# WHU-USI3DV/LaneMapping

Hardware: AMD Instinct MI355X
Metric: BEV tiles/sec end-to-end (LAS points -> polylines) (higher is better)
Workload: dtype f32

## Files before the change

include/lanemap_hip.h:

```cpp
#ifndef LANEMAP_HIP_H
#define LANEMAP_HIP_H
#include <stdint.h>
#ifdef __cplusplus
extern "C" {
#endif

enum { LM_OK = 0, LM_ERR_ARG = 1, LM_ERR_HIP = 2, LM_ERR_NO_DEVICE = 3 };
enum { LM_ACT_NONE = 0, LM_ACT_RELU = 1, LM_ACT_GELU = 2 };

int lm_abi_version(void);
const char* lm_last_error(void);
int lm_device_count(void);

int lm_conv2d_nhwc_mfma_f32(void* stream, const float* x, int ldx, const float* wp, int CoutP,
                            const float* scale, const float* shift, const float* res, int ldr, int res_rows,
                            float* y, int ldy, int B, int H, int W, int Cin, int Cout, int KH, int KW,
                            int stride, int pad_h, int pad_w, int dil, int act);
int lm_conv2d_nhwc_mfma_resup_f32(void* stream, const float* x, int ldx, const float* wp, int CoutP, const float* scale,
                                  const float* shift, const float* res_coarse, int ldr, int Hr, int Wr, float* y, int ldy,
                                  int B, int H, int W, int Cin, int Cout, int KH, int KW, int stride, int pad_h, int pad_w,
                                  int dil, int act);

int lm_winograd44_supported(int H, int W, int Cin, int dil);
int lm_winograd44_gn_chunks(int H, int W, int dil);
long lm_winograd44_tiles(int B, int H, int W, int dil);
long lm_winograd44_twin_workspace_bytes(int B, int H, int W, int Cin, int CoutP, int dil);
int lm_conv3x3_winograd44_f32(void* stream, const float* x, int ldx, const float* wu_frag, int CoutP, const float* scale,
                              const float* shift, const float* res, int ldr, float* y, int ldy, int B, int H, int W,
                              int Cin, int Cout, int dil, int act, double* gn_partial);
int lm_conv3x3_winograd44_twin_f32(void* stream, const float* x, int ldx, const float* wu, int CoutP, const float* scale,
                                   const float* shift, const float* res, int ldr, float* y, int ldy, int B, int H, int W,
                                   int Cin, int Cout, int dil, int act, void* workspace, long workspace_bytes);
int lm_wino44_split_fragments(void* stream, const float* frag, float* out, long n_quads);
int lm_conv3x3_winograd44_split_f32(void* stream, const float* x, int ldx, const float* wu_split, int CoutP, const float* scale,
                                    const float* shift, const float* res, int ldr, float* y, int ldy, int B, int H, int W,
                                    int Cin, int Cout, int dil, int act, double* gn_partial, float post);
int lm_conv3x3_winograd44_split_twin_f32(void* stream, const float* x, int ldx, const float* wu, int CoutP, const float* scale,
                                         const float* shift, const float* res, int ldr, float* y, int ldy, int B, int H, int W,
// ... 151 lines not shown
```

lanemapping_amd/_lib.py:

```python
import ctypes as C
import os

_HERE = os.path.dirname(os.path.abspath(__file__))
LIB_PATH = os.environ.get('LANEMAP_HIP_LIB') or os.path.join(_HERE, 'liblanemap_hip.so')

c_f32p = C.POINTER(C.c_float)
vp, i32, i64, f32 = C.c_void_p, C.c_int, C.c_long, C.c_float


class LmRasterParams(C.Structure):
    _fields_ = [('quat', C.c_float * 4), ('trans', C.c_float * 3), ('bev_img_offset', C.c_float * 2),
                ('img_reso', C.c_float * 2), ('local_min_ele', C.c_float), ('ele_reso', C.c_float),
                ('inten_lo', C.c_float), ('inten_hi', C.c_float)]


class LmLasHeader(C.Structure):
    _fields_ = [('version_major', C.c_int), ('version_minor', C.c_int), ('point_format', C.c_int), ('record_len', C.c_int),
                ('n_points', C.c_long), ('offset_to_points', C.c_long), ('scale', C.c_double * 3), ('offset', C.c_double * 3),
                ('min_xyz', C.c_double * 3), ('max_xyz', C.c_double * 3)]


SIGNATURES = {
    'lm_abi_version': (i32, []),
    'lm_last_error': (C.c_char_p, []),
    'lm_device_count': (i32, []),
    'lm_conv2d_nhwc_mfma_f32': (i32, [vp, vp, i32, vp, i32, vp, vp, vp, i32, i32, vp, i32,
                                      i32, i32, i32, i32, i32, i32, i32, i32, i32, i32, i32, i32]),
    'lm_conv2d_nhwc_mfma_resup_f32': (i32, [vp, vp, i32, vp, i32, vp, vp, vp, i32, i32, i32, vp, i32,
                                            i32, i32, i32, i32, i32, i32, i32, i32, i32, i32, i32, i32]),
    'lm_winograd44_supported': (i32, [i32, i32, i32, i32]),
    'lm_winograd44_gn_chunks': (i32, [i32, i32, i32]),
    'lm_winograd44_tiles': (i64, [i32, i32, i32, i32]),
    'lm_winograd44_twin_workspace_bytes': (i64, [i32, i32, i32, i32, i32, i32]),
    'lm_conv3x3_winograd44_f32': (i32, [vp, vp, i32, vp, i32, vp, vp, vp, i32, vp, i32, i32, i32, i32, i32, i32, i32, i32, vp]),
    'lm_conv3x3_winograd44_twin_f32': (i32, [vp, vp, i32, vp, i32, vp, vp, vp, i32, vp, i32, i32, i32, i32, i32, i32, i32, i32, vp, i64]),
    'lm_wino44_split_fragments': (i32, [vp, vp, vp, i64]),
    'lm_conv3x3_winograd44_split_f32': (i32, [vp, vp, i32, vp, i32, vp, vp, vp, i32, vp, i32, i32, i32, i32, i32, i32, i32, i32, vp, f32]),
    'lm_conv3x3_winograd44_split_twin_f32': (i32, [vp, vp, i32, vp, i32, vp, vp, vp, i32, vp, i32, i32, i32, i32, i32, i32, i32, i32, vp, i64, f32]),
    'lm_conv2d_nhwc_mfma_f32_gnstats': (i32, [vp, vp, i32, vp, i32, vp, vp, i32, vp] + [i32] * 11),
    'lm_gn_finalize': (i32, [vp, vp, vp, i32, i32, i32, i32, f32]),
    'lm_gn_finalize_split': (i32, [vp, vp, vp, i32, i32, i32, i32, f32, i32]),
    'lm_stem_conv7x7_bn_relu': (i32, [vp, vp, vp, vp, vp, vp, i32, i32, i32]),
    'lm_stem_conv7x7_bn_relu_u8': (i32, [vp, vp, vp, vp, vp, vp, i32, i32, i32]),
    'lm_maxpool3x3s2_nhwc': (i32, [vp, vp, vp, i32, i32, i32, i32]),
    'lm_conv2d_nhwc_small': (i32, [vp, vp, i32, vp, vp, vp, vp, i32, i32, i32, i32, i32, i32, i32, i32, i32, i32, i32, i32, i32]),
    'lm_gn_stats': (i32, [vp, vp, vp, vp, i32, i32, i32, f32]),
# ... 95 lines not shown
```

lanemapping_amd/csrc/conv_wino44.hip:

```cpp
#include "common.h"

#include <cstdlib>

typedef float f32x16 __attribute__((ext_vector_type(16)));
typedef float f32x4 __attribute__((ext_vector_type(4)));
typedef float f32x2 __attribute__((ext_vector_type(2)));
typedef _Float16 f16x4 __attribute__((ext_vector_type(4)));
typedef unsigned u32x2 __attribute__((ext_vector_type(2)));

namespace {

__device__ __forceinline__ u32x2 w44_split2(f32x2 t) {
#pragma clang fp contract(off)
    typedef __fp16 f16x2r __attribute__((ext_vector_type(2)));
    const f16x2r h = __builtin_amdgcn_cvt_pkrtz(t[0], t[1]);
    const float h0 = (float)h[0], h1 = (float)h[1];
    const f16x2r l = __builtin_amdgcn_cvt_pkrtz(t[0] - h0, t[1] - h1);
    return u32x2{__builtin_bit_cast(unsigned, h), __builtin_bit_cast(unsigned, l)};
}

constexpr int QBM = 32, QBN = 64, QSEG = 4;
constexpr int QNCELL = 144;
constexpr int QLPW = 14;
constexpr int QGRP = 256 + 8;
constexpr int QRAWF = QLPW * 4 * QGRP;
constexpr int QVF = 36 * 256;
constexpr int QBD = 5, QRING = 6;
static_assert(6 * (QNCELL / 16) * QGRP <= QRAWF && QNCELL % 16 == 0, "patch loads cover the unit");

__device__ __attribute__((aligned(16))) float g_w44_zeros[1024 + 32];

struct W44Geom {
    int B, H, W, dil, Ty, Tx;
    int Timg, Tpad;
    long T;
    LmFastDiv dTx, dTy, ddil, dTpad;
};

W44Geom geom44(int B, int H, int W, int dil) {
    W44Geom g;
    g.B = B; g.H = H; g.W = W; g.dil = dil;
    g.Ty = ((H + dil - 1) / dil + 3) / 4;
    g.Tx = ((W + dil - 1) / dil + 3) / 4;
    g.Timg = dil * dil * g.Ty * g.Tx;
    g.Tpad = (g.Timg + QBM - 1) / QBM * QBM;
    g.T = (long)B * g.Tpad;
    g.dTx = lm_fastdiv_make((unsigned)g.Tx); g.dTy = lm_fastdiv_make((unsigned)g.Ty);
    g.ddil = lm_fastdiv_make((unsigned)dil); g.dTpad = lm_fastdiv_make((unsigned)g.Tpad);
    return g;
}

__device__ __forceinline__ void tile44_decode(const W44Geom& g, int t, int& pa, int& pb, int& ty, int& tx) {
    tx = t % g.Tx;
    t /= g.Tx;
    ty = t % g.Ty;
    const int ph = t / g.Ty;
    pa = ph / g.dil;
    pb = ph - pa * g.dil;
}

// ... 188 lines not shown
    const f32x2 p = pk_fnma(d[2], k.c4, d[4]), q = pk_fnma(d[1], k.c4, d[3]);
    const f32x2 r = pk_sub(d[4], d[2]), s = pk_sub(d[3], d[1]);
    t[0] = pk_fma(d[0], k.c4, a);
    t[5] = pk_fma(d[1], k.c4, b);
    t[1] = pk_add(p, q);
    t[2] = pk_sub(p, q);
    t[3] = pk_fma(s, k.c2, r);
    t[4] = pk_fnma(s, k.c2, r);
}

struct W44Xf {
    f32x2 e[6][5];
    f32x2 w[3][6];
    f32x2 tA[6], tB[6], tC[6];
};
template <int C>
__device__ __forceinline__ void w44_preread(W44Xf& d, const float* rawrow, const int (&roff)[6]) {
    constexpr int ROWF = (QNCELL / 16) * QGRP;
    const float* s = rawrow + roff[C];
#pragma unroll
    for (int r = 0; r < 5; ++r) d.e[C][r] = *reinterpret_cast<const f32x2*>(s + r * ROWF);
}
template <bool LOWER, int C>
__device__ __forceinline__ void w44_pass1x2(W44Xf& d, const W44K& k) {
    const f32x2 (&e)[5] = d.e[C];
    const f32x2 (&f)[5] = d.e[C + 1];
    if constexpr (!LOWER) {
        const f32x2 a0 = pk_fnma(e[2], k.c5, e[4]), a1 = pk_fnma(f[2], k.c5, f[4]);
        const f32x2 p0 = pk_fnma(e[2], k.c4, e[4]), p1 = pk_fnma(f[2], k.c4, f[4]);
        const f32x2 q0 = pk_fnma(e[1], k.c4, e[3]), q1 = pk_fnma(f[1], k.c4, f[3]);
        d.w[0][C] = pk_fma(e[0], k.c4, a0);
        d.w[0][C + 1] = pk_fma(f[0], k.c4, a1);
        d.w[1][C] = pk_add(p0, q0);
        d.w[1][C + 1] = pk_add(p1, q1);
        d.w[2][C] = pk_sub(p0, q0);
        d.w[2][C + 1] = pk_sub(p1, q1);
    } else {
        const f32x2 a0 = pk_fnma(e[2], k.c5, e[4]), a1 = pk_fnma(f[2], k.c5, f[4]);
        const f32x2 r0 = pk_sub(e[3], e[1]), r1 = pk_sub(f[3], f[1]);
        const f32x2 s0 = pk_sub(e[2], e[0]), s1 = pk_sub(f[2], f[0]);
        d.w[2][C] = pk_fma(e[0], k.c4, a0);
        d.w[2][C + 1] = pk_fma(f[0], k.c4, a1);
        d.w[0][C] = pk_fma(s0, k.c2, r0);
        d.w[0][C + 1] = pk_fma(s1, k.c2, r1);
        d.w[1][C] = pk_fnma(s0, k.c2, r0);
        d.w[1][C + 1] = pk_fnma(s1, k.c2, r1);
    }
}
template <bool SPLIT>
__device__ __forceinline__ void w44_vstore(float* v, int j, const f32x2 t) {
    if constexpr (SPLIT) {
        const u32x2 w = w44_split2(t);
        reinterpret_cast<unsigned*>(v)[j * 256] = w[0];
        reinterpret_cast<unsigned*>(v)[j * 256 + 128] = w[1];
    } else {
        *reinterpret_cast<f32x2*>(v + j * 256) = t;
    }
}
template <int K, bool SPLIT>
__device__ __forceinline__ void w44_xf_lds(W44Xf& d, const float* rawrow, const int (&roff)[6], float* vA, float* vB, float* vC) {
    auto st = [](float* v, int j, const f32x2 t) { w44_vstore<SPLIT>(v, j, t); };
    if constexpr (K == 0) {
        st(vB, 2, d.tB[2]); st(vB, 5, d.tB[5]);
        w44_preread<0>(d, rawrow, roff); w44_preread<1>(d, rawrow, roff);
    } else if constexpr (K == 1) {
        st(vC, 0, d.tC[0]); st(vC, 1, d.tC[1]);
        w44_preread<2>(d, rawrow, roff); w44_preread<3>(d, rawrow, roff);
    } else if constexpr (K == 2) {
        st(vC, 2, d.tC[2]); st(vC, 3, d.tC[3]);
        w44_preread<4>(d, rawrow, roff); w44_preread<5>(d, rawrow, roff);
    } else if constexpr (K == 3) {
        st(vC, 4, d.tC[4]); st(vC, 5, d.tC[5]);
    } else if constexpr (K == 5) {
        st(vA, 0, d.tA[0]); st(vA, 1, d.tA[1]); st(vA, 2, d.tA[2]);
    } else if constexpr (K == 6) {
        st(vA, 3, d.tA[3]); st(vA, 4, d.tA[4]); st(vA, 5, d.tA[5]);
    } else if constexpr (K == 7) {
        st(vB, 0, d.tB[0]); st(vB, 1, d.tB[1]); st(vB, 3, d.tB[3]); st(vB, 4, d.tB[4]);
    }
}
template <int K>
__device__ __forceinline__ void w44_xf_valu(W44Xf& d, bool lower, const W44K& k) {
    if constexpr (K >= 1 && K <= 3) {
        if (lower) w44_pass1x2<true, 2 * K - 2>(d, k);
        else w44_pass1x2<false, 2 * K - 2>(d, k);
    } else if constexpr (K == 4) {
        pk_bt(d.w[0], d.tA, k);
    } else if constexpr (K == 5) {
        pk_bt(d.w[1], d.tB, k);
    } else if constexpr (K == 6) {
        pk_bt(d.w[2], d.tC, k);
    }
}
template <bool SPLIT>
__device__ __forceinline__ void w44_xf_all(W44Xf& d, const float* rawrow, const int (&roff)[6], float* vA, float* vB, float* vC, bool lower,
                                           const W44K& k) {
    w44_preread<0>(d, rawrow, roff); w44_preread<1>(d, rawrow, roff); w44_preread<2>(d, rawrow, roff);
    w44_preread<3>(d, rawrow, roff); w44_preread<4>(d, rawrow, roff); w44_preread<5>(d, rawrow, roff);
    w44_xf_valu<1>(d, lower, k); w44_xf_valu<2>(d, lower, k); w44_xf_valu<3>(d, lower, k);
    w44_xf_valu<4>(d, lower, k); w44_xf_valu<5>(d, lower, k); w44_xf_valu<6>(d, lower, k);
#pragma unroll
    for (int j = 0; j < 6; ++j) {
        w44_vstore<SPLIT>(vA, j, d.tA[j]);
        w44_vstore<SPLIT>(vB, j, d.tB[j]);
        w44_vstore<SPLIT>(vC, j, d.tC[j]);
    }
}

__device__ __forceinline__ void q_bload2(f32x4 (&b)[2], unsigned voff, const float* sbase) {
    asm volatile("global_load_dwordx4 %0, %2, %3\n\t"
                 "global_load_dwordx4 %1, %2, %3 offset:1024"
                 : "=&v"(b[0]), "=&v"(b[1]) : "v"(voff), "s"(sbase) : "memory");
}
template <int N>
__device__ __forceinline__ void q_bwait(f32x4 (&b)[2]) {
    asm volatile("s_waitcnt vmcnt(%2)" : "+v"(b[0]), "+v"(b[1]) : "n"(N) : "memory");
}

__device__ __forceinline__ void mfma_vgpr(f32x16& acc, float a, float b) {
    asm volatile("v_mfma_f32_32x32x2_f32 %0, %1, %2, %0" : "+v"(acc) : "v"(a), "v"(b));
// ... 38 lines not shown
    constexpr int K = S % 9;
    q_bload2(bq[(S + QBD) % QRING], bvoff, bpre);
#pragma unroll
    for (int i = 0; i < q_ndma(S); ++i) {
        constexpr int L0 = q_dma0(S);
        __builtin_amdgcn_global_load_lds((gptr_t*)(gsrc[L0 + i] + goff), (lptr_t*)(rawld + ((L0 + i) * 4 + wave) * QGRP), 16, 0, 0);
    }
    f32x4 (&b)[2] = bq[S % QRING];
    q_bwait<q_nwait(S)>(b);
    constexpr bool VACC = K == 8;
    const f32x2 a_hi = {a_cur[0], a_cur[1]}, a_lo = {a_cur[2], a_cur[3]};
    if constexpr (SPLIT) q_mfma16<VACC>(acc0, a_hi, f32x2{b[0][0], b[0][1]});
    else q_mfma<VACC>(acc0, a_cur[0], b[0][0]);
    if constexpr (!SPLIT) __builtin_amdgcn_sched_barrier(0);
    if constexpr (K != 4 && K != 8) a_nxt = q_aread<SPLIT>(anext);
    w44_xf_lds<K, SPLIT>(xf, prerow, roff, vA, vB, vC);
    if constexpr (!SPLIT) __builtin_amdgcn_sched_barrier(0);
    w44_xf_valu<K>(xf, lower, kk);
    if constexpr (!SPLIT) __builtin_amdgcn_sched_barrier(0);
    if constexpr (SPLIT) {
        q_mfma16<VACC>(acc1, a_hi, f32x2{b[1][0], b[1][1]});
        q_mfma16<VACC>(acc0, a_hi, f32x2{b[0][2], b[0][3]});
        q_mfma16<VACC>(acc1, a_hi, f32x2{b[1][2], b[1][3]});
        q_mfma16<VACC>(acc0, a_lo, f32x2{b[0][0], b[0][1]});
        q_mfma16<VACC>(acc1, a_lo, f32x2{b[1][0], b[1][1]});
        if constexpr (!VACC) {
#pragma unroll
            for (int i = 0; i < 6; ++i) {
                __builtin_amdgcn_sched_group_barrier(0x008, 1, 0);
                __builtin_amdgcn_sched_group_barrier(0x002, 6, 0);
                __builtin_amdgcn_sched_group_barrier(0x300, 3, 0);
// ... 182 lines not shown
            for (int r = 0; r < 16; ++r) acc[k][b][r] = 0.f;
    f32x4 bq[QRING][2];
    W44Xf xf;
    const int lowoff = lower ? (QNCELL / 16) * QGRP : 0;
#define LM_QXI(K) (6 * ((K) / 3) + (K) % 3)
#pragma unroll
    for (int k = 0; k < QBD; ++k) q_bload2(bq[k], bvoff, bbase + (long)LM_QXI(k) * xstride);
    {
        const long goff1 = nun > 1 ? 16 : 0;
#pragma unroll
        for (int s_ = 0; s_ < QLPW; ++s_)
            __builtin_amdgcn_global_load_lds((gptr_t*)(gsrc[s_] + goff1), (lptr_t*)(raw0 + QRAWF + (s_ * 4 + wave) * QGRP), 16, 0, 0);
    }
    q_bwait<QLPW>(bq[0]);
    __builtin_amdgcn_s_barrier();
    w44_xf_all<SPLIT>(xf, raw0 + lowoff, roff, vA, vB, vC, lower, kk);
    asm volatile("s_waitcnt lgkmcnt(0)" ::: "memory");
    __builtin_amdgcn_s_barrier();

#define LM_QBPRE(S5) ((S5) < 18 ? bu + (long)((S5) / 9) * ustride + (long)LM_QXI((S5) % 9) * xstride : bu_next + (long)LM_QXI((S5) - 18) * xstride)
#define LM_QSTEP(S, AC, AN) \
    w44_step<S, SPLIT>(acc[(S) % 9][0], acc[(S) % 9][1], bq, bvoff, LM_QBPRE((S) + QBD), Vq + LM_QXI(((S) % 9) + 1 < 9 ? ((S) % 9) + 1 : 0) * 256, \
                AC, AN, gsrc, goff, rawc_w, wave, xf, (S) < 9 ? rawc + 8 + lowoff : rawn + lowoff, roff, vA, vB, vC, lower, kk)
#define LM_QMID(AN)                                          \
    asm volatile("s_waitcnt lgkmcnt(0)" ::: "memory");       \
    __builtin_amdgcn_s_barrier();                            \
    AN = q_aread<SPLIT>(Vq + LM_QXI(5) * 256);
    for (int u = 0; u < nun; ++u) {
        const float* const rawc = raw0 + (u & 1) * QRAWF;
        float* const rawc_w = raw0 + (u & 1) * QRAWF;
        const float* const rawn = raw0 + ((u + 1) & 1) * QRAWF;
// ... 156 lines not shown
                const f32x4 b = *reinterpret_cast<const f32x4*>(smem + (((w * 2 + blk) * 8 + cq) * 2 + 1) * 4);
#pragma unroll
                for (int e = 0; e < 4; ++e) {
                    s[e] += a[e];
                    q[e] += b[e];
                }
            }
            const long chunk = t0 / 32;
            double* o = p.gn_part + (((long)bi * (g.Tpad / 32) + chunk) * p.Cout + n) * 2;
            for (int e = 0; e < 4 && n + e < p.Cout; ++e) {
                o[2 * e] = (double)s[e];
                o[2 * e + 1] = (double)q[e];
            }
        }
    }
}

bool w44_ok(const W44Geom& g) { return (QBM - 2) / g.Tx + 2 <= QSEG; }

int w44_zeros(const float** out) {
    static const float* cache[64] = {nullptr};
    int dev = 0;
    LM_HIP(hipGetDevice(&dev));
    LM_REQUIRE(dev >= 0 && dev < 64, "conv_wino44: device index %d", dev);
    if (!cache[dev]) {
        void* sym = nullptr;
        LM_HIP(hipGetSymbolAddress(&sym, HIP_SYMBOL(g_w44_zeros)));
        cache[dev] = (const float*)sym;
    }
    *out = cache[dev];
// ... 39 lines not shown
    static_assert(36 * 32 * 32 <= 2 * QRAWF + QVF, "the product buffer of the epilogue fits");
    const long blocks = (p.g.T / QBM) * ((Cout + QBN - 1) / QBN);
    LM_REQUIRE(blocks > 0 && blocks < (1L << 31) && p.g.T % QBM == 0, "conv_wino44: bad grid %ld", blocks);
    p.post = split_post != 0.f ? split_post : 1.f;
    if (split_post != 0.f) {
        if (int e = lm_ensure_dynamic_lds((const void*)wino44_kernel<true>, lds)) return e;
        hipLaunchKernelGGL(wino44_kernel<true>, dim3((unsigned)blocks), dim3(256), lds, (hipStream_t)stream, p);
    } else {
        if (int e = lm_ensure_dynamic_lds((const void*)wino44_kernel<false>, lds)) return e;
        hipLaunchKernelGGL(wino44_kernel<false>, dim3((unsigned)blocks), dim3(256), lds, (hipStream_t)stream, p);
    }
    LM_LAUNCH_CHECK();
    return LM_OK;
}

LM_API int lm_conv3x3_winograd44_f32(void* stream, const float* x, int ldx, const float* wu_frag, int CoutP, const float* scale,
                                     const float* shift, const float* res, int ldr, float* y, int ldy, int B, int H, int W,
                                     int Cin, int Cout, int dil, int act, double* gn_partial) {
    return w44_launch(stream, x, ldx, wu_frag, CoutP, scale, shift, res, ldr, y, ldy, B, H, W, Cin, Cout, dil, act, gn_partial, 0.f);
}

LM_API int lm_conv3x3_winograd44_split_f32(void* stream, const float* x, int ldx, const float* wu_split, int CoutP, const float* scale,
                                           const float* shift, const float* res, int ldr, float* y, int ldy, int B, int H, int W,
                                           int Cin, int Cout, int dil, int act, double* gn_partial, float post) {
    LM_REQUIRE(post > 0.f, "conv_wino44(split): post scale must be positive");
    return w44_launch(stream, x, ldx, wu_split, CoutP, scale, shift, res, ldr, y, ldy, B, H, W, Cin, Cout, dil, act, gn_partial, post);
}

LM_API int lm_wino44_split_fragments(void* stream, const float* frag, float* out, long n_quads) {
    LM_REQUIRE(frag && out && n_quads > 0 && n_quads < (1L << 38), "wino44_split_fragments: bad arguments");
    hipLaunchKernelGGL(wino44_split_frag_kernel, dim3((unsigned)((n_quads + 255) / 256)), dim3(256), 0, (hipStream_t)stream,
                       reinterpret_cast<const f32x4*>(frag), reinterpret_cast<f32x4*>(out), n_quads);
    LM_LAUNCH_CHECK();
// ... 47 lines not shown
```

lanemapping_amd/ops.py:

```python
import ctypes as C
import math

import torch

from ._lib import lib, check, LmRasterParams, LanemapHipError

ACT_NONE, ACT_RELU, ACT_GELU = 0, 1, 2


def _stream():
    return C.c_void_p(torch._C._cuda_getCurrentRawStream(torch._C._cuda_getDevice()))


def _ptr(t):
    if t is None:
        return None
    if not t.is_cuda:
        raise LanemapHipError('lanemapping_amd ops need tensors on an MI355X (HIP) device; no CPU fallback exists')
    if t.device.index != torch._C._cuda_getDevice():
        raise LanemapHipError(f'tensor on cuda:{t.device.index} but the current device is cuda:{torch._C._cuda_getDevice()}: '
                              'call torch.cuda.set_device() (one process drives one GPU)')
    return C.c_void_p(t.data_ptr())


# ... 38 lines not shown
    co, ci, kh, kw = w.shape
    assert kh == 3 and kw == 3
    G = torch.tensor(_W44_G, device=w.device, dtype=torch.float64)
    U = torch.einsum('ij,ocjk,lk->iloc', G, w.double(), G).reshape(36, co, ci).float()
    cop = (co + 63) // 64 * 64
    p = torch.zeros((36, cop, ci), device=w.device, dtype=torch.float32)
    p[:, :co, :] = U
    return p.contiguous()


def pack_wino44_fragments(wu):
    xi, cop, ci = wu.shape
    assert xi == 36 and cop % 64 == 0 and ci % 16 == 0
    t = wu.reshape(36, cop // 32, 32, ci // 8, 2, 4)
    return t.permute(0, 3, 1, 4, 2, 5).contiguous().reshape(36, ci // 8, cop // 32, 64, 4)


class SplitFragments:
    __slots__ = ('words', 'post')

    def __init__(self, words, post):
        self.words, self.post = words, float(post)

    @property
    def shape(self):
        return self.words.shape


def split_scale(wu):
    m = float(wu.abs().max())
# ... 74 lines not shown
def _hooked(kind, flops, launch, executed=None):
    if _conv_hook is not None:
        _conv_hook(kind, flops, launch, executed)
    else:
        launch()


def wino44_supported(H, W, cin, dil=1):
    return bool(lib().lm_winograd44_supported(int(H), int(W), int(cin), int(dil)))


def conv_wino44(x, wf, cout, dil=1, scale=None, shift=None, res=None, act=ACT_NONE, out=None, gn_eps=None, gn_split=1):
    x, ldx = as_nhwc(x)
    B, cin, H, W = x.shape
    cop = wf.shape[2] * 32
    y = out if out is not None else new_act(B, cout, H, W, x.device)
    y_, ldy = as_nhwc(y)
    assert y_.data_ptr() == y.data_ptr(), 'conv_wino44: `out` must already be NHWC-stored'
    r, ldr = (None, 0) if res is None else as_nhwc(res)
    part = None
    if gn_eps is not None:
        part = torch.empty((B, lib().lm_winograd44_gn_chunks(H, W, dil), cout, 2), device=x.device, dtype=torch.float64)
    tiles = lib().lm_winograd44_tiles(B, H, W, dil)
    if isinstance(wf, SplitFragments):
        _hooked(f'wino44split {cin}->{cout} k3x3 d{dil} @{H}x{W} B{B}', 2.0 * B * H * W * cout * cin * 9,
                lambda: check(lib().lm_conv3x3_winograd44_split_f32(_stream(), _ptr(x), ldx, _ptr(wf.words), cop, _ptr(scale), _ptr(shift), _ptr(r),
                                                                    ldr, _ptr(y), ldy, B, H, W, cin, cout, dil, act, _ptr(part), wf.post)),
                3 * 2.0 * 36 * tiles * cin * cout)
    else:
        _hooked(f'wino44 {cin}->{cout} k3x3 d{dil} @{H}x{W} B{B}', 2.0 * B * H * W * cout * cin * 9,
# ... 540 lines not shown
```

lanemapping_amd/pcencoder.py:

```python
import os

import torch
import torch.nn as nn

from . import ops, trace
from .registry import PCENCODER
from .packing import PackedModule

_LAYERS = {'resnet18': [2, 2, 2, 2], 'resnet34': [3, 4, 6, 3]}
MERGE_BRANCH_CONVS = os.environ.get('LANEMAP_MERGE_BRANCH_CONVS', '1') != '0'
WINO_F44 = os.environ.get('LANEMAP_WINO_F44', '1') != '0'
WINO_F44_MIN_CIN = int(os.environ.get('LANEMAP_WINO_F44_MIN_CIN', '64'))
WINO_SPLIT = os.environ.get('LANEMAP_WINO_SPLIT', '0') != '0'


def _frag44(w):
    if WINO_SPLIT:
        return ops.pack_wino44_fragments_split(ops.pack_wino44(w))
    return ops.pack_wino44_fragments(ops.pack_wino44(w))


def _f44_ok(conv):
    return WINO_F44 and conv.kernel_size == (3, 3) and conv.stride == (1, 1) and conv.in_channels >= WINO_F44_MIN_CIN and conv.in_channels % 16 == 0


class _ResBlock(nn.Module):

    def __init__(self, cin, cout, stride, dilation, with_down):
        super().__init__()
        self.conv1 = nn.Conv2d(cin, cout, 3, stride, dilation, dilation, bias=False)
        self.bn1 = nn.BatchNorm2d(cout)
        self.conv2 = nn.Conv2d(cout, cout, 3, 1, dilation, dilation, bias=False)
        self.bn2 = nn.BatchNorm2d(cout)
# ... 80 lines not shown
                P[k + '.s1'], P[k + '.b1'] = ops.fold_bn(blk.bn1)
                P[k + '.w2'] = ops.pack_mfma(blk.conv2.weight)
                P[k + '.s2'], P[k + '.b2'] = ops.fold_bn(blk.bn2)
                for q, conv in (('.w1q', blk.conv1), ('.w2q', blk.conv2)):
                    if _f44_ok(conv):
                        P[k + q] = _frag44(conv.weight)
                if blk.downsample is not None:
                    P[k + '.wd'] = ops.pack_mfma(blk.downsample[0].weight)
                    P[k + '.sd'], P[k + '.bd'] = ops.fold_bn(blk.downsample[1])
        for name in ('toplayer', 'smooth1', 'smooth2', 'smooth3', 'latlayer1', 'latlayer2', 'semantic_branch',
                     'semantic_branch2', 'conv2', 'conv3'):
            m = getattr(self, name)
            P[name + '.w'] = ops.pack_mfma(m.weight)
            P[name + '.b'] = m.bias.float().contiguous()
            if _f44_ok(m):
                P[name + '.wq'] = _frag44(m.weight)
        a, b2 = self.semantic_branch, self.semantic_branch2
        if (MERGE_BRANCH_CONVS and 'semantic_branch.wq' in P and 'semantic_branch2.wq' in P and a.out_channels == b2.out_channels
                and self.gn11.eps == self.gn21.eps):
            P['semantic_branch_ab.wq'] = _frag44(torch.cat([a.weight, b2.weight], dim=0))
            P['semantic_branch_ab.b'] = torch.cat([a.bias, b2.bias]).float().contiguous()
            if ('conv2.wq' in P and 'conv3.wq' in P and self.conv2.out_channels == self.conv3.out_channels
                    and self.gn12.eps == self.gn22.eps):
                P['conv23.wq'] = _frag44(torch.cat([self.conv2.weight, self.conv3.weight], dim=0))
                P['conv23.b'] = torch.cat([self.conv2.bias, self.conv3.bias]).float().contiguous()
        if self.out is not None:
            P['out.w'] = ops.pack_mfma(self.out.weight)
        for name in ('feature_layer', 'output_layer_binary_seg', 'output_layer_endp'):
            m = getattr(self, name)
            P[name + '.w'] = ops.pack_small(m.weight)
            P[name + '.b'] = m.bias.float().contiguous()
        for name in ('gn11', 'gn12', 'gn21', 'gn22'):
            m = getattr(self, name)
            P[name + '.g'], P[name + '.b'] = m.weight.float().contiguous(), m.bias.float().contiguous()
        return P

    @staticmethod
    def _c3(x, P, wkey, cout, stride, dil, **epi):
        if (wkey + 'q') in P and stride == 1 and ops.wino44_supported(x.shape[2], x.shape[3], x.shape[1], dil):
# ... 114 lines not shown
```

Measured before the change: 394.4.

## Add Winograd F(4,3) kernel variant with 16x128 tiles for wide-Cout convs

```diff
diff --git a/include/lanemap_hip.h b/include/lanemap_hip.h
--- a/include/lanemap_hip.h
+++ b/include/lanemap_hip.h
@@ -22,6 +22,7 @@
                                   int dil, int act);
 
 int lm_winograd44_supported(int H, int W, int Cin, int dil);
+int lm_winograd44_n128(int Cout, int gn);
 int lm_winograd44_gn_chunks(int H, int W, int dil);
 long lm_winograd44_tiles(int B, int H, int W, int dil);
 long lm_winograd44_twin_workspace_bytes(int B, int H, int W, int Cin, int CoutP, int dil);
diff --git a/lanemapping_amd/_lib.py b/lanemapping_amd/_lib.py
--- a/lanemapping_amd/_lib.py
+++ b/lanemapping_amd/_lib.py
@@ -30,6 +30,7 @@
                                             i32, i32, i32, i32, i32, i32, i32, i32, i32, i32, i32, i32]),
     'lm_winograd44_supported': (i32, [i32, i32, i32, i32]),
     'lm_winograd44_gn_chunks': (i32, [i32, i32, i32]),
+    'lm_winograd44_n128': (i32, [i32, i32]),
     'lm_winograd44_tiles': (i64, [i32, i32, i32, i32]),
     'lm_winograd44_twin_workspace_bytes': (i64, [i32, i32, i32, i32, i32, i32]),
     'lm_conv3x3_winograd44_f32': (i32, [vp, vp, i32, vp, i32, vp, vp, vp, i32, vp, i32, i32, i32, i32, i32, i32, i32, i32, vp]),
diff --git a/lanemapping_amd/csrc/conv_wino44.hip b/lanemapping_amd/csrc/conv_wino44.hip
--- a/lanemapping_amd/csrc/conv_wino44.hip
+++ b/lanemapping_amd/csrc/conv_wino44.hip
@@ -37,13 +37,13 @@
     LmFastDiv dTx, dTy, ddil, dTpad;
 };
 
-W44Geom geom44(int B, int H, int W, int dil) {
+W44Geom geom44(int B, int H, int W, int dil, int mblk = QBM) {
     W44Geom g;
     g.B = B; g.H = H; g.W = W; g.dil = dil;
     g.Ty = ((H + dil - 1) / dil + 3) / 4;
     g.Tx = ((W + dil - 1) / dil + 3) / 4;
     g.Timg = dil * dil * g.Ty * g.Tx;
-    g.Tpad = (g.Timg + QBM - 1) / QBM * QBM;
+    g.Tpad = (g.Timg + mblk - 1) / mblk * mblk;
     g.T = (long)B * g.Tpad;
     g.dTx = lm_fastdiv_make((unsigned)g.Tx); g.dTy = lm_fastdiv_make((unsigned)g.Ty);
     g.ddil = lm_fastdiv_make((unsigned)dil); g.dTpad = lm_fastdiv_make((unsigned)g.Tpad);
@@ -262,9 +262,8 @@
     f32x2 w[3][6];
     f32x2 tA[6], tB[6], tC[6];
 };
-template <int C>
+template <int C, int ROWF = (QNCELL / 16) * QGRP>
 __device__ __forceinline__ void w44_preread(W44Xf& d, const float* rawrow, const int (&roff)[6]) {
-    constexpr int ROWF = (QNCELL / 16) * QGRP;
     const float* s = rawrow + roff[C];
 #pragma unroll
     for (int r = 0; r < 5; ++r) d.e[C][r] = *reinterpret_cast<const f32x2*>(s + r * ROWF);
@@ -295,28 +294,32 @@
         d.w[1][C + 1] = pk_fnma(s1, k.c2, r1);
     }
 }
-template <bool SPLIT>
+enum { W44V_PAIR = 0, W44V_SPLIT = 1, W44V_N128 = 2 };
+template <int VS>
 __device__ __forceinline__ void w44_vstore(float* v, int j, const f32x2 t) {
-    if constexpr (SPLIT) {
+    if constexpr (VS == W44V_SPLIT) {
         const u32x2 w = w44_split2(t);
         reinterpret_cast<unsigned*>(v)[j * 256] = w[0];
         reinterpret_cast<unsigned*>(v)[j * 256 + 128] = w[1];
+    } else if constexpr (VS == W44V_N128) {
+        v[j * 256] = t[0];
+        v[j * 256 + 128] = t[1];
     } else {
         *reinterpret_cast<f32x2*>(v + j * 256) = t;
     }
 }
-template <int K, bool SPLIT>
+template <int K, int VS, int ROWF = (QNCELL / 16) * QGRP>
 __device__ __forceinline__ void w44_xf_lds(W44Xf& d, const float* rawrow, const int (&roff)[6], float* vA, float* vB, float* vC) {
-    auto st = [](float* v, int j, const f32x2 t) { w44_vstore<SPLIT>(v, j, t); };
+    auto st = [](float* v, int j, const f32x2 t) { w44_vstore<VS>(v, j, t); };
     if constexpr (K == 0) {
         st(vB, 2, d.tB[2]); st(vB, 5, d.tB[5]);
-        w44_preread<0>(d, rawrow, roff); w44_preread<1>(d, rawrow, roff);
+        w44_preread<0, ROWF>(d, rawrow, roff); w44_preread<1, ROWF>(d, rawrow, roff);
     } else if constexpr (K == 1) {
         st(vC, 0, d.tC[0]); st(vC, 1, d.tC[1]);
-        w44_preread<2>(d, rawrow, roff); w44_preread<3>(d, rawrow, roff);
+        w44_preread<2, ROWF>(d, rawrow, roff); w44_preread<3, ROWF>(d, rawrow, roff);
     } else if constexpr (K == 2) {
         st(vC, 2, d.tC[2]); st(vC, 3, d.tC[3]);
-        w44_preread<4>(d, rawrow, roff); w44_preread<5>(d, rawrow, roff);
+        w44_preread<4, ROWF>(d, rawrow, roff); w44_preread<5, ROWF>(d, rawrow, roff);
     } else if constexpr (K == 3) {
         st(vC, 4, d.tC[4]); st(vC, 5, d.tC[5]);
     } else if constexpr (K == 5) {
@@ -340,18 +343,18 @@
         pk_bt(d.w[2], d.tC, k);
     }
 }
-template <bool SPLIT>
+template <int VS, int ROWF = (QNCELL / 16) * QGRP>
 __device__ __forceinline__ void w44_xf_all(W44Xf& d, const float* rawrow, const int (&roff)[6], float* vA, float* vB, float* vC, bool lower,
                                            const W44K& k) {
-    w44_preread<0>(d, rawrow, roff); w44_preread<1>(d, rawrow, roff); w44_preread<2>(d, rawrow, roff);
-    w44_preread<3>(d, rawrow, roff); w44_preread<4>(d, rawrow, roff); w44_preread<5>(d, rawrow, roff);
+    w44_preread<0, ROWF>(d, rawrow, roff); w44_preread<1, ROWF>(d, rawrow, roff); w44_preread<2, ROWF>(d, rawrow, roff);
+    w44_preread<3, ROWF>(d, rawrow, roff); w44_preread<4, ROWF>(d, rawrow, roff); w44_preread<5, ROWF>(d, rawrow, roff);
     w44_xf_valu<1>(d, lower, k); w44_xf_valu<2>(d, lower, k); w44_xf_valu<3>(d, lower, k);
     w44_xf_valu<4>(d, lower, k); w44_xf_valu<5>(d, lower, k); w44_xf_valu<6>(d, lower, k);
 #pragma unroll
     for (int j = 0; j < 6; ++j) {
-        w44_vstore<SPLIT>(vA, j, d.tA[j]);
-        w44_vstore<SPLIT>(vB, j, d.tB[j]);
-        w44_vstore<SPLIT>(vC, j, d.tC[j]);
+        w44_vstore<VS>(vA, j, d.tA[j]);
+        w44_vstore<VS>(vB, j, d.tB[j]);
+        w44_vstore<VS>(vC, j, d.tC[j]);
     }
 }
 
@@ -420,7 +423,7 @@
     else q_mfma<VACC>(acc0, a_cur[0], b[0][0]);
     if constexpr (!SPLIT) __builtin_amdgcn_sched_barrier(0);
     if constexpr (K != 4 && K != 8) a_nxt = q_aread<SPLIT>(anext);
-    w44_xf_lds<K, SPLIT>(xf, prerow, roff, vA, vB, vC);
+    w44_xf_lds<K, SPLIT ? W44V_SPLIT : W44V_PAIR>(xf, prerow, roff, vA, vB, vC);
     if constexpr (!SPLIT) __builtin_amdgcn_sched_barrier(0);
     w44_xf_valu<K>(xf, lower, kk);
     if constexpr (!SPLIT) __builtin_amdgcn_sched_barrier(0);
@@ -633,7 +636,7 @@
     }
     q_bwait<QLPW>(bq[0]);
     __builtin_amdgcn_s_barrier();
-    w44_xf_all<SPLIT>(xf, raw0 + lowoff, roff, vA, vB, vC, lower, kk);
+    w44_xf_all<SPLIT ? W44V_SPLIT : W44V_PAIR>(xf, raw0 + lowoff, roff, vA, vB, vC, lower, kk);
     asm volatile("s_waitcnt lgkmcnt(0)" ::: "memory");
     __builtin_amdgcn_s_barrier();
 
@@ -820,6 +823,361 @@
             }
         }
     }
+}
+
+constexpr int NBM = 16, NBN = 128;
+constexpr int NGRP = 5;
+constexpr int NLPW = 8;
+constexpr int NROWF = NGRP * QGRP;
+constexpr int NRAWF = NLPW * 4 * QGRP;
+constexpr int NMLD = 68, NMXI = NBM * NMLD;
+constexpr int NSM = 36 * NMXI;
+constexpr int NBD = 2, NRING = 3;
+static_assert(6 * NGRP <= 4 * NLPW && 2 * NRAWF + QVF <= NSM, "patch loads cover the unit; raw + V buffers fit");
+static_assert(18 % NRING == 0 && NBD < NRING, "eighteen half steps per unit walk the ring a whole number of times");
+
+__device__ __forceinline__ void n_bload4(f32x4 (&b)[4], unsigned voff, const float* sbase) {
+    asm volatile("global_load_dwordx4 %0, %4, %5\n\t"
+                 "global_load_dwordx4 %1, %4, %5 offset:1024\n\t"
+                 "global_load_dwordx4 %2, %4, %5 offset:2048\n\t"
+                 "global_load_dwordx4 %3, %4, %5 offset:3072"
+                 : "=&v"(b[0]), "=&v"(b[1]), "=&v"(b[2]), "=&v"(b[3]) : "v"(voff), "s"(sbase) : "memory");
+}
+template <int N>
+__device__ __forceinline__ void n_bwait(f32x4 (&b)[4]) {
+    asm volatile("s_waitcnt vmcnt(%4)" : "+v"(b[0]), "+v"(b[1]), "+v"(b[2]), "+v"(b[3]) : "n"(N) : "memory");
+}
+template <bool VACC>
+__device__ __forceinline__ void n_mfma(f32x4& acc, float a, float b) {
+    if constexpr (VACC) asm volatile("v_mfma_f32_16x16x4_f32 %0, %1, %2, %0" : "+v"(acc) : "v"(a), "v"(b));
+    else asm volatile("v_mfma_f32_16x16x4_f32 %0, %1, %2, %0" : "+a"(acc) : "v"(a), "v"(b));
+}
+constexpr int n_ndma(int H) { return H < NLPW ? 1 : 0; }
+constexpr int n_nwait(int H) {
+    int c = 0;
+    for (int j = H - NBD; j <= H; ++j) c += n_ndma(((j % 18) + 18) % 18);
+    return 4 * NBD + c;
+}
+constexpr int n_nafter() {
+    int c = 0;
+    for (int j = NLPW; j < 18; ++j) c += 4;
+    return c;
+}
+static_assert(n_nafter() < 64 && n_nwait(0) < 64, "vmcnt range");
+
+template <int H>
+__device__ __forceinline__ void n_half(f32x4 (&acc)[8], f32x4 (&bq)[NRING][4], unsigned bvoff, const float* bpre, const float* anext,
+                                       const f32x4& a_cur, f32x4& a_nxt, const float* const (&gsrc)[NLPW], long goff, float* rawld, int wave,
+                                       W44Xf& xf, const float* prerow, const int (&roff)[6], float* vA, float* vB, float* vC, bool lower,
+                                       const W44K& kk) {
+    typedef __attribute__((address_space(1))) const void gptr_t;
+    typedef __attribute__((address_space(3))) void lptr_t;
+    constexpr int K = H / 2, h = H % 2;
+    constexpr bool VACC = K == 8;
+    n_bload4(bq[(H + NBD) % NRING], bvoff, bpre);
+    if constexpr (n_ndma(H) > 0)
+        __builtin_amdgcn_global_load_lds((gptr_t*)(gsrc[H] + goff), (lptr_t*)(rawld + (H * 4 + wave) * QGRP), 16, 0, 0);
+    f32x4 (&b)[4] = bq[H % NRING];
+    n_bwait<n_nwait(H)>(b);
+    n_mfma<VACC>(acc[0], a_cur[2 * h], b[0][0]);
+    if constexpr (h == 0) {
+        __builtin_amdgcn_sched_barrier(0);
+        if constexpr (K != 4 && K != 8) a_nxt = *reinterpret_cast<const f32x4*>(anext);
+        w44_xf_lds<K, W44V_N128, NROWF>(xf, prerow, roff, vA, vB, vC);
+        __builtin_amdgcn_sched_barrier(0);
+        w44_xf_valu<K>(xf, lower, kk);
+    }
+    __builtin_amdgcn_sched_barrier(0);
+#pragma unroll
+    for (int t = 0; t < 2; ++t)
+#pragma unroll
+        for (int nb = t == 0 ? 1 : 0; nb < 8; ++nb) n_mfma<VACC>(acc[nb], a_cur[2 * h + t], b[nb >> 1][2 * (nb & 1) + t]);
+    __builtin_amdgcn_sched_barrier(0);
+}
+
+__global__ __launch_bounds__(256) void wino44n_kernel(W44Params p) {
+    extern __shared__ __attribute__((aligned(16))) float smem[];
+    float* const raw0 = smem;
+    float* const Vbuf = smem + 2 * NRAWF;
+    typedef __attribute__((address_space(1))) const void gptr_t;
+    typedef __attribute__((address_space(3))) void lptr_t;
+    const int tid = threadIdx.x, lane = tid & 63;
+    const int wave = __builtin_amdgcn_readfirstlane(tid >> 6);
+    const int n_tiles = (p.Cout + NBN - 1) / NBN;
+    unsigned mblk, ntile;
+    if (p.n_inner) {
+        const unsigned bid = blockIdx.x, per = gridDim.x / 8;
+        const unsigned lin = bid < per * 8 ? (bid % 8) * per + bid / 8 : bid;
+        mblk = lm_fastdiv(lin, p.dnt);
+        ntile = lin - mblk * (unsigned)n_tiles;
+    } else {
+        const unsigned bid = blockIdx.x, mb = gridDim.x / (unsigned)n_tiles, mbx = mb / 8, full = mbx * 8 * (unsigned)n_tiles;
+        if (bid < full) {
+            const unsigned xcd = bid % 8, idx = bid / 8;
+            ntile = idx / mbx;
+            mblk = xcd * mbx + idx % mbx;
+        } else {
+            const unsigned r = bid - full;
+            mblk = 8 * mbx + r / (unsigned)n_tiles;
+            ntile = r % (unsigned)n_tiles;
+        }
+    }
+    const long m0 = (long)mblk * NBM;
+    const int n0 = (int)ntile * NBN;
+    const W44Geom& g = p.g;
+    const int bi = (int)lm_fastdiv((unsigned)m0, g.dTpad);
+    const int t0 = (int)(m0 - (long)bi * g.Tpad);
+    int ts[QSEG + 1], sn[QSEG], iy0[QSEG], ix0[QSEG], oy0[QSEG], ox0[QSEG];
+    {
+        int at = 0, t = t0;
+        const int rest = (int)lm_fastdiv((unsigned)t0, g.dTx), ph = (int)lm_fastdiv((unsigned)rest, g.dTy);
+        int tx = t0 - rest * g.Tx, ty = rest - ph * g.Ty;
+        int pa = (int)lm_fastdiv((unsigned)ph, g.ddil), pb = ph - pa * g.dil;
+#pragma unroll
+        for (int s_ = 0; s_ < QSEG; ++s_) {
+            ts[s_] = at;
+            const bool real = t < g.Timg && at < NBM;
+            const int n = at < NBM ? min(NBM - at, g.Tx - tx) : 0;
+            sn[s_] = real ? n : 0;
+            iy0[s_] = (4 * ty - 1) * g.dil + pa;
+            ix0[s_] = (4 * tx - 1) * g.dil + pb;
+            oy0[s_] = 4 * ty * g.dil + pa;
+            ox0[s_] = 4 * tx * g.dil + pb;
+            at += n;
+            t += n;
+            tx += n;
+            if (tx >= g.Tx) {
+                tx = 0;
+                if (++ty >= g.Ty) {
+                    ty = 0;
+                    if (++pb >= g.dil) {
+                        pb = 0;
+                        ++pa;
+                    }
+                }
+            }
+        }
+        ts[QSEG] = at;
+    }
+    const float* gsrc[NLPW];
+    const int img_pix0 = bi * g.H * g.W;
+    int tab_x, tab_y, tab_n;
+    {
+        int n = sn[0], yb = iy0[0], xb = ix0[0], s0 = 0;
+#pragma unroll
+        for (int k = 1; k < QSEG; ++k) {
+            const bool in = lane >= ts[k] + k;
+            n = in ? sn[k] : n;
+            yb = in ? iy0[k] : yb;
+            xb = in ? ix0[k] : xb;
+            s0 = in ? ts[k] + k : s0;
+        }
+        const int j = lane - s0;
+        tab_x = xb + 4 * j * g.dil;
+        tab_y = yb;
+        tab_n = n > 0 ? 4 * (n - j) + 2 : 0;
+    }
+    const int gcc = (lane >> 4) & 3, gccd = gcc * g.dil, gsl4 = ((lane >> 2) & 3) << 2, gcq4 = (lane & 3) * 4;
+#pragma unroll
+    for (int s_ = 0; s_ < NLPW; ++s_) {
+        const int q = s_ * 4 + wave;
+        const int r = q / NGRP, gq = q - r * NGRP;
+        const int idx = 16 * gq + gsl4;
+        const int x0 = __builtin_amdgcn_ds_bpermute(idx, tab_x), y0 = __builtin_amdgcn_ds_bpermute(idx, tab_y);
+        const int nn = __builtin_amdgcn_ds_bpermute(idx, tab_n);
+        const int yy = y0 + r * g.dil, xx = x0 + gccd;
+        const bool ok = (r < 6) & (gcc < nn) & ((unsigned)yy < (unsigned)g.H) & ((unsigned)xx < (unsigned)g.W);
+        const long m = -(long)ok;
+        const long eoff = ((long)(img_pix0 + yy * g.W + xx) * p.ldx) & m;
+        const unsigned long base = (unsigned long)p.zeros + (((unsigned long)p.x - (unsigned long)p.zeros) & (unsigned long)m);
+        gsrc[s_] = (const float*)base + eoff + gcq4;
+        __builtin_amdgcn_global_load_lds((gptr_t*)gsrc[s_], (lptr_t*)(raw0 + (s_ * 4 + wave) * QGRP), 16, 0, 0);
+        __builtin_amdgcn_sched_barrier(0);
+    }
+    int roff[6], tvoff;
+    {
+        const int tl = lane & 15;
+        int sg = 0;
+#pragma unroll
+        for (int k = 1; k < QSEG; ++k) sg += (ts[k] < NBM && tl >= ts[k]) ? 1 : 0;
+        const int slot = tl + sg, slot1 = slot + 1;
+        const int cp = ((lane >> 4) + 4 * (wave & 1) + 2 * slot) & 7;
+        const int pos0 = 16 * (slot >> 2) + (slot & 3), pos1 = 16 * (slot1 >> 2) + (slot1 & 3);
+#pragma unroll
+        for (int c = 0; c < 6; ++c) {
+            const int pos = c < 4 ? pos0 + 4 * c : pos1 + 4 * (c - 4);
+            roff[c] = (pos >> 4) * QGRP + (pos & 15) * 16 + 2 * cp;
+        }
+        tvoff = ((cp >> 1) & 1) * 64 + tl * 4 + 2 * (cp >> 2) + (cp & 1);
+    }
+    const bool lower = (wave >> 1) != 0;
+    float* const vA = Vbuf + (lower ? 3 : 0) * (6 * 256) + tvoff;
+    float* const vB = Vbuf + (lower ? 4 : 1) * (6 * 256) + tvoff;
+    float* const vC = Vbuf + (lower ? 5 : 2) * (6 * 256) + tvoff;
+    const W44K kk = {f32x2{2.f, 2.f}, f32x2{4.f, 4.f}, f32x2{5.f, 5.f}};
+    const int qa = wave >> 1, qb = wave & 1;
+    const int xi00 = 18 * qa + 3 * qb;
+    const float* const Vq = Vbuf + xi00 * 256 + lane * 4;
+    const int nun = p.C / 16;
+    const unsigned bvoff = (unsigned)lane * 16u;
+    const long ustride = (long)p.NT * 256;
+    const long xstride = (long)(2 * nun) * ustride;
+    const float* const bbase = p.U + (long)xi00 * xstride + (long)(n0 >> 5) * 256;
+
+    f32x4 acc[9][8];
+#pragma unroll
+    for (int k = 0; k < 9; ++k)
+#pragma unroll
+        for (int b = 0; b < 8; ++b) acc[k][b] = f32x4{0.f, 0.f, 0.f, 0.f};
+    f32x4 bq[NRING][4];
+    W44Xf xf;
+    const int lowoff = lower ? NROWF : 0;
+#define LM_NXI(K) (6 * ((K) / 3) + (K) % 3)
+#pragma unroll
+    for (int k = 0; k < NBD; ++k) n_bload4(bq[k], bvoff, bbase + (long)(k & 1) * ustride);
+    {
+        const long goff1 = nun > 1 ? 16 : 0;
+#pragma unroll
+        for (int s_ = 0; s_ < NLPW; ++s_)
+            __builtin_amdgcn_global_load_lds((gptr_t*)(gsrc[s_] + goff1), (lptr_t*)(raw0 + NRAWF + (s_ * 4 + wave) * QGRP), 16, 0, 0);
+    }
+    n_bwait<NLPW>(bq[0]);
+    __builtin_amdgcn_s_barrier();
+    w44_xf_all<W44V_N128, NROWF>(xf, raw0 + lowoff, roff, vA, vB, vC, lower, kk);
+    n_bwait<0>(bq[0]);
+    asm volatile("s_waitcnt lgkmcnt(0)" ::: "memory");
+    __builtin_amdgcn_s_barrier();
+
+#define LM_NBPRE(H2) ((H2) < 18 ? bu + (long)((H2) & 1) * ustride + (long)LM_NXI((H2) / 2) * xstride \
+                                : bu_next + (long)((H2) & 1) * ustride + (long)LM_NXI(((H2) - 18) / 2) * xstride)
+#define LM_NHALF(H, AC, AN) \
+    n_half<H>(acc[(H) / 2], bq, bvoff, LM_NBPRE((H) + NBD), Vq + LM_NXI((H) / 2 + 1 < 9 ? (H) / 2 + 1 : 0) * 256, AC, AN, gsrc, goff, rawc_w, \
+              wave, xf, rawn + lowoff, roff, vA, vB, vC, lower, kk)
+#define LM_NSTEP(K, AC, AN) LM_NHALF(2 * (K), AC, AN); LM_NHALF(2 * (K) + 1, AC, AN);
+    for (int u = 0; u < nun; ++u) {
+        float* const rawc_w = raw0 + (u & 1) * NRAWF;
+        const float* const rawn = raw0 + ((u + 1) & 1) * NRAWF;
+        const long goff = u + 2 < nun ? (long)(u + 2) * 16 : 0;
+        const float* const bu = bbase + (long)(2 * u) * ustride;
+        const float* const bu_next = bbase + (long)(u + 1 < nun ? 2 * (u + 1) : 0) * ustride;
+        f32x4 a0, a1;
+        a0 = *reinterpret_cast<const f32x4*>(Vq);
+        LM_NSTEP(0, a0, a1) LM_NSTEP(1, a1, a0) LM_NSTEP(2, a0, a1) LM_NSTEP(3, a1, a0) LM_NSTEP(4, a0, a1)
+        asm volatile("s_waitcnt lgkmcnt(0)" ::: "memory");
+        __builtin_amdgcn_s_barrier();
+        a1 = *reinterpret_cast<const f32x4*>(Vq + LM_NXI(5) * 256);
+        LM_NSTEP(5, a1, a0) LM_NSTEP(6, a0, a1) LM_NSTEP(7, a1, a0) LM_NSTEP(8, a0, a1)
+        n_bwait<n_nafter()>(bq[0]);
+        asm volatile("s_waitcnt lgkmcnt(0)" ::: "memory");
+        __builtin_amdgcn_s_barrier();
+    }
+#undef LM_NSTEP
+#undef LM_NHALF
+#undef LM_NBPRE
+#pragma unroll
+    for (int k = 0; k < NRING; ++k) n_bwait<0>(bq[k]);
+    asm volatile("s_nop 15\n\ts_nop 15" ::: "memory");
+
+    const int etile = tid >> 4, ecq = tid & 15;
+    int epix0;
+    int eny = 0, enx = 0;
+    {
+        int nn = sn[0], oy = oy0[0], oxb = ox0[0], tb = 0;
+#pragma unroll
+        for (int k = 1; k < QSEG; ++k)
+            if (etile >= ts[k]) {
+                nn = sn[k]; oy = oy0[k]; oxb = ox0[k]; tb = ts[k];
+            }
+        const int ox = oxb + 4 * (etile - tb) * g.dil;
+        epix0 = img_pix0 + oy * g.W + ox;
+        if (nn > 0 && oy < g.H && ox < g.W) {
+            eny = min(4, (int)lm_fastdiv((unsigned)(g.H - oy + g.dil - 1), g.ddil));
+            enx = min(4, (int)lm_fastdiv((unsigned)(g.W - ox + g.dil - 1), g.ddil));
+        }
+    }
+    float* const mw = smem + xi00 * NMXI + 4 * (lane >> 4) * NMLD + (lane & 15);
+    const float* const mr = smem + etile * NMLD + ecq * 4;
+    const bool full = eny == 4 && enx == 4;
+    const int ebase = eny > 0 ? epix0 : img_pix0;
+    const int ey1 = max(eny - 1, 0), ex1 = max(enx - 1, 0);
+    const float relu_lo = p.act == LM_ACT_RELU ? 0.f : -__builtin_inff();
+    const bool has_res = p.res != nullptr;
+    f32x4 gdummy = {0.f, 0.f, 0.f, 0.f};
+#pragma unroll
+    for (int rnd = 0; rnd < 2; ++rnd) {
+        const int n = n0 + rnd * 64 + ecq * 4;
+        const bool vec = (n + 3 < p.Cout) && ((p.ldy & 3) == 0) && (!p.res || (p.ldr & 3) == 0);
+        f32x4 sc = {1.f, 1.f, 1.f, 1.f}, sh = {0.f, 0.f, 0.f, 0.f};
+        if (vec) {
+            if (p.scale) sc = *reinterpret_cast<const f32x4*>(p.scale + n);
+            if (p.shift) sh = *reinterpret_cast<const f32x4*>(p.shift + n);
+        } else {
+#pragma unroll
+            for (int e = 0; e < 4; ++e)
+                if (n + e < p.Cout) {
+                    if (p.scale) sc[e] = p.scale[n + e];
+                    if (p.shift) sh[e] = p.shift[n + e];
+                }
+        }
+        f32x4 rpre[16];
+        const bool load_res = vec && has_res;
+        const float* const rp = p.res + (long)ebase * p.ldr + n;
+        const int rs = g.W * g.dil * p.ldr, cs = g.dil * p.ldr;
+        asm volatile("s_waitcnt lgkmcnt(0)" ::: "memory");
+        __builtin_amdgcn_s_barrier();
+#pragma unroll
+        for (int k = 0; k < 9; ++k) {
+#pragma unroll
+            for (int b = 0; b < 4; ++b)
+#pragma unroll
+                for (int r = 0; r < 4; ++r) mw[LM_NXI(k) * NMXI + r * NMLD + b * 16] = acc[k][4 * rnd + b][r];
+            if (k < 8 && load_res) {
+#pragma unroll
+                for (int q = 2 * k; q < 2 * k + 2; ++q)
+                    rpre[q] = *reinterpret_cast<const f32x4*>(rp + min(q >> 2, ey1) * rs + min(q & 3, ex1) * cs);
+            }
+            __builtin_amdgcn_sched_barrier(0);
+        }
+        asm volatile("s_waitcnt lgkmcnt(0)" ::: "memory");
+        __builtin_amdgcn_s_barrier();
+        if (n < p.Cout && eny > 0) {
+            f32x4 z[4][6];
+#pragma unroll
+            for (int j = 0; j < 6; ++j) {
+                f32x4 col[6], y4[4];
+#pragma unroll
+                for (int i = 0; i < 6; ++i) col[i] = *reinterpret_cast<const f32x4*>(mr + (6 * i + j) * NMXI);
+                w44_at(col, y4);
+#pragma unroll
+                for (int yy = 0; yy < 4; ++yy) z[yy][j] = y4[yy];
+            }
+            float* const yp = p.y + (long)ebase * p.ldy + n;
+            const int rowstep = g.W * g.dil * p.ldy, colstep = g.dil * p.ldy;
+            if (vec) {
+                if (full) w44_tail_vec<true>(z, rpre, yp, rowstep, colstep, sc, sh, relu_lo, has_res, false, gdummy, gdummy, eny, enx);
+                else w44_tail_vec<false>(z, rpre, yp, rowstep, colstep, sc, sh, relu_lo, has_res, false, gdummy, gdummy, eny, enx);
+            } else {
+#pragma unroll
+                for (int yy = 0; yy < 4; ++yy) {
+                    f32x4 o[4];
+                    w44_at(z[yy], o);
+#pragma unroll
+                    for (int xx = 0; xx < 4; ++xx) {
+#pragma clang fp contract(off)
+                        const f32x4 v = o[xx] * sc + sh;
+#pragma unroll
+                        for (int e = 0; e < 4; ++e) {
+                            if (!(yy < eny && xx < enx && n + e < p.Cout)) continue;
+                            float uu = v[e];
+                            if (has_res) uu += p.res[((long)ebase + (yy * g.W + xx) * g.dil) * p.ldr + n + e];
+                            yp[yy * rowstep + xx * colstep + e] = fmaxf(uu, relu_lo);
+                        }
+                    }
+                }
+            }
+        }
+    }
+#undef LM_NXI
 }
 
 bool w44_ok(const W44Geom& g) { return (QBM - 2) / g.Tx + 2 <= QSEG; }
@@ -889,9 +1247,48 @@
     return LM_OK;
 }
 
+static bool w44_n128_enabled() {
+    static const bool on = !getenv("LANEMAP_W44_N128") || atoi(getenv("LANEMAP_W44_N128")) != 0;
+    return on;
+}
+
+LM_API int lm_winograd44_n128(int Cout, int gn) { return w44_n128_enabled() && Cout >= NBN && !gn ? 1 : 0; }
+
+static int w44n_launch(void* stream, const float* x, int ldx, const float* wu_frag, int CoutP, const float* scale, const float* shift,
+                       const float* res, int ldr, float* y, int ldy, int B, int H, int W, int Cin, int Cout, int dil, int act,
+                       double* gn_partial) {
+    LM_REQUIRE(x && wu_frag && y, "conv_wino44n: null pointer");
+    LM_REQUIRE(lm_winograd44_n128(Cout, gn_partial != nullptr), "conv_wino44n: fragments packed for wino44n_kernel, but Cout=%d%s does not "
+               "run there (LANEMAP_W44_N128=0, Cout < %d or GroupNorm statistics)", Cout, gn_partial ? " + gn stats" : "", NBN);
+    LM_REQUIRE(lm_winograd44_supported(H, W, Cin, dil) && B > 0, "conv_wino44n: unsupported shape (H=%d W=%d Cin=%d dil=%d)", H, W, Cin, dil);
+    LM_REQUIRE(CoutP >= Cout && CoutP % NBN == 0, "conv_wino44n: CoutP=%d must be Cout=%d rounded up to %d", CoutP, Cout, NBN);
+    LM_REQUIRE(ldx >= Cin && ldx % 4 == 0 && ldy >= Cout, "conv_wino44n: bad leading dimension");
+    LM_REQUIRE(act == LM_ACT_NONE || act == LM_ACT_RELU, "conv_wino44n: activation %d not supported", act);
+    W44Params p;
+    p.g = geom44(B, H, W, dil, NBM);
+    LM_REQUIRE((long)B * H * W * ldx < (1L << 40) && (long)B * H * W < (1L << 31) && p.g.T < (1L << 31), "conv_wino44n: tensor too large");
+    p.x = x; p.U = wu_frag; p.scale = scale; p.shift = shift; p.res = res; p.y = y;
+    p.ldx = ldx; p.ldr = ldr; p.ldy = ldy; p.C = Cin; p.Cout = Cout; p.NT = CoutP / 32; p.act = act;
+    p.gn_part = nullptr;
+    p.post = 1.f;
+    if (int e = w44_zeros(&p.zeros)) return e;
+    static const int order = getenv("LANEMAP_W44_ORDER") ? atoi(getenv("LANEMAP_W44_ORDER")) : 1;
+    p.n_inner = order;
+    p.dnt = lm_fastdiv_make((unsigned)((Cout + NBN - 1) / NBN));
+    const size_t lds = (size_t)NSM * sizeof(float);
+    const long blocks = (p.g.T / NBM) * ((Cout + NBN - 1) / NBN);
+    LM_REQUIRE(blocks > 0 && blocks < (1L << 31) && p.g.T % NBM == 0, "conv_wino44n: bad grid %ld", blocks);
+    if (int e = lm_ensure_dynamic_lds((const void*)wino44n_kernel, lds)) return e;
+    hipLaunchKernelGGL(wino44n_kernel, dim3((unsigned)blocks), dim3(256), lds, (hipStream_t)stream, p);
+    LM_LAUNCH_CHECK();
+    return LM_OK;
+}
+
 LM_API int lm_conv3x3_winograd44_f32(void* stream, const float* x, int ldx, const float* wu_frag, int CoutP, const float* scale,
                                      const float* shift, const float* res, int ldr, float* y, int ldy, int B, int H, int W,
                                      int Cin, int Cout, int dil, int act, double* gn_partial) {
+    if (CoutP < 0)
+        return w44n_launch(stream, x, ldx, wu_frag, -CoutP, scale, shift, res, ldr, y, ldy, B, H, W, Cin, Cout, dil, act, gn_partial);
     return w44_launch(stream, x, ldx, wu_frag, CoutP, scale, shift, res, ldr, y, ldy, B, H, W, Cin, Cout, dil, act, gn_partial, 0.f);
 }
 
diff --git a/lanemapping_amd/ops.py b/lanemapping_amd/ops.py
--- a/lanemapping_amd/ops.py
+++ b/lanemapping_amd/ops.py
@@ -76,6 +76,31 @@
     assert xi == 36 and cop % 64 == 0 and ci % 16 == 0
     t = wu.reshape(36, cop // 32, 32, ci // 8, 2, 4)
     return t.permute(0, 3, 1, 4, 2, 5).contiguous().reshape(36, ci // 8, cop // 32, 64, 4)
+
+
+class N128Fragments:
+    __slots__ = ('frag',)
+
+    def __init__(self, frag):
+        self.frag = frag
+
+    @property
+    def shape(self):
+        return self.frag.shape
+
+
+def wino44_n128(cout, gn=False):
+    return bool(lib().lm_winograd44_n128(int(cout), 1 if gn else 0))
+
+
+def pack_wino44_fragments16(wu):
+    xi, cop, ci = wu.shape
+    assert xi == 36 and cop % 64 == 0 and ci % 16 == 0
+    cop2 = (cop + 127) // 128 * 128
+    if cop2 != cop:
+        wu = torch.cat([wu, wu.new_zeros((36, cop2 - cop, ci))], dim=1)
+    t = wu.reshape(36, cop2 // 32, 2, 16, ci // 8, 2, 2, 2)
+    return N128Fragments(t.permute(0, 4, 1, 7, 5, 3, 2, 6).contiguous().reshape(36, ci // 8, cop2 // 32, 64, 4))
 
 
 class SplitFragments:
@@ -180,6 +205,8 @@
     x, ldx = as_nhwc(x)
     B, cin, H, W = x.shape
     cop = wf.shape[2] * 32
+    if isinstance(wf, N128Fragments):
+        wf, cop = wf.frag, -cop
     y = out if out is not None else new_act(B, cout, H, W, x.device)
     y_, ldy = as_nhwc(y)
     assert y_.data_ptr() == y.data_ptr(), 'conv_wino44: `out` must already be NHWC-stored'
diff --git a/lanemapping_amd/pcencoder.py b/lanemapping_amd/pcencoder.py
--- a/lanemapping_amd/pcencoder.py
+++ b/lanemapping_amd/pcencoder.py
@@ -14,9 +14,14 @@
 WINO_SPLIT = os.environ.get('LANEMAP_WINO_SPLIT', '0') != '0'
 
 
-def _frag44(w):
+_GN_CONVS = ('semantic_branch', 'semantic_branch2', 'conv2', 'conv3')
+
+
+def _frag44(w, gn=False):
     if WINO_SPLIT:
         return ops.pack_wino44_fragments_split(ops.pack_wino44(w))
+    if ops.wino44_n128(w.shape[0], gn):
+        return ops.pack_wino44_fragments16(ops.pack_wino44(w))
     return ops.pack_wino44_fragments(ops.pack_wino44(w))
 
 
@@ -127,15 +132,15 @@
             P[name + '.w'] = ops.pack_mfma(m.weight)
             P[name + '.b'] = m.bias.float().contiguous()
             if _f44_ok(m):
-                P[name + '.wq'] = _frag44(m.weight)
+                P[name + '.wq'] = _frag44(m.weight, gn=name in _GN_CONVS)
         a, b2 = self.semantic_branch, self.semantic_branch2
         if (MERGE_BRANCH_CONVS and 'semantic_branch.wq' in P and 'semantic_branch2.wq' in P and a.out_channels == b2.out_channels
                 and self.gn11.eps == self.gn21.eps):
-            P['semantic_branch_ab.wq'] = _frag44(torch.cat([a.weight, b2.weight], dim=0))
+            P['semantic_branch_ab.wq'] = _frag44(torch.cat([a.weight, b2.weight], dim=0), gn=True)
             P['semantic_branch_ab.b'] = torch.cat([a.bias, b2.bias]).float().contiguous()
             if ('conv2.wq' in P and 'conv3.wq' in P and self.conv2.out_channels == self.conv3.out_channels
                     and self.gn12.eps == self.gn22.eps):
-                P['conv23.wq'] = _frag44(torch.cat([self.conv2.weight, self.conv3.weight], dim=0))
+                P['conv23.wq'] = _frag44(torch.cat([self.conv2.weight, self.conv3.weight], dim=0), gn=True)
                 P['conv23.b'] = torch.cat([self.conv2.bias, self.conv3.bias]).float().contiguous()
         if self.out is not None:
             P['out.w'] = ops.pack_mfma(self.out.weight)
```

After: 397.8, median of 6. No clear change (+0.9%).
